# HybridRobotics/car-racing

Measured on AMD Instinct MI355X. Metric: NLP solves/sec (N=12, 6-state bicycle); p50 per-step solve latency, higher is better.
Workload: dtype f64

## Files before the change

### car-racing_amd/csrc/crx_api.hip

```cpp
#include <hip/hip_runtime.h>
#include <math.h>
#include <stdarg.h>
#include <stdio.h>
#include <string.h>

#include <dlfcn.h>

#include <chrono>
#include <mutex>
#include <vector>

#if __has_include(<rccl/rccl.h>)
#include <rccl/rccl.h>
#else
extern "C" {
typedef struct ncclComm* ncclComm_t;
typedef struct { char internal[128]; } ncclUniqueId;
typedef enum { ncclSuccess = 0 } ncclResult_t;
typedef enum { ncclInt8 = 0, ncclUint8 = 1, ncclInt32 = 2, ncclUint32 = 3, ncclInt64 = 4, ncclUint64 = 5, ncclFloat16 = 6, ncclFloat32 = 7, ncclFloat64 = 8 } ncclDataType_t;
}
#endif

#include "crx_kparams.h"

// ... 35 lines not shown
    }
    void release() {
        if (p) (void)hipFree(p);
        p = nullptr;
        cap = 0;
    }
};
DevBuf g_in, g_out;

struct PinBuf {
    void* p = nullptr;
    size_t cap = 0;
    int ensure(size_t bytes) {
        if (bytes <= cap) return 0;
        if (p) (void)hipHostFree(p);
        p = nullptr;
        cap = 0;
        size_t want = bytes + bytes / 2 + 256;
        hipError_t e = hipHostMalloc(&p, want, hipHostMallocDefault);
        if (e != hipSuccess) return fail(CRX_ERR_HIP, "hipHostMalloc(%zu): %s", want, hipGetErrorString(e));
        cap = want;
        return 0;
    }
    void release() {
        if (p) (void)hipHostFree(p);
        p = nullptr;
        cap = 0;
    }
};
PinBuf g_hin, g_hout;
DevBuf g_trace;
int g_poison = 0;
int g_kkt_unscaled = 0;
int g_spec = 0;
int g_trace_rows = 0, g_trace_problem = 0;

int ensure_init() {
    if (g_init) return 0;
    return fail(CRX_ERR_NOT_INIT, "crx_init() has not been called (or failed)");
}

struct Stage {
    size_t oi = 0, oo = 0;
    struct Back { void* host; size_t off, bytes; };
    Back backs[16];
    int nb = 0;
    int reserve(size_t bytes_in, size_t bytes_out) {
        bytes_in += 20 * 256; bytes_out += 20 * 256;
        if (int rc = g_in.ensure(bytes_in)) return rc;
        if (int rc = g_hin.ensure(bytes_in)) return rc;
        if (int rc = g_out.ensure(bytes_out)) return rc;
        return g_hout.ensure(bytes_out);
    }
    template <typename T>
    T* in(const T* src, size_t n) {
        oi = (oi + 255) & ~size_t(255);
        T* dev = (T*)((char*)g_in.p + oi);
        if (n) {
            if (src) memcpy((char*)g_hin.p + oi, src, n * sizeof(T)); else memset((char*)g_hin.p + oi, 0, n * sizeof(T));
        }
        oi += n * sizeof(T);
        return dev;
    }
    template <typename T>
    T* out(T* host, size_t n) {
        oo = (oo + 255) & ~size_t(255);
// ... 81 lines not shown
    memcpy(kp.wq, d->Q, sizeof(kp.wq)); kp.wr[0] = d->R[0]; kp.wr[1] = d->R[1];
    kp.w_dey = 0.0; kp.w_prog = 0.0; kp.w_slack = d->w_slack;
    kp.delta_max = d->delta_max; kp.a_max = d->a_max; kp.v_min = d->v_min; kp.v_max = d->v_max; kp.ey_max = d->ey_max;
    kp.alpha = d->alpha; kp.margin = d->margin; kp.l_sum = d->l_sum; kp.w_sum = d->w_sum;
    kp.dt_ref = 0.1; kp.fallback_gain = 1.1; kp.opts = d->opts;
    kp.slack_start = d->opts.slack_start;
    double ws[6] = {0, 0, 0, 0, 1, 0}, we[6] = {0, 0, 0, 0, 0, 1}, as = 0.0, ae = 0.0;
    kp.reach_s[0] = 0.0; kp.reach_gain[0] = 0.0;
    for (int j = 1; j <= d->N; j++) {
        double s0 = 0.0, s1 = 0.0, e0 = 0.0, e1 = 0.0, wn[6] = {0, 0, 0, 0, 0, 0}, en[6] = {0, 0, 0, 0, 0, 0};
        for (int i = 0; i < 6; i++) {
            s0 += ws[i] * d->B[i * 2]; s1 += ws[i] * d->B[i * 2 + 1];
            e0 += we[i] * d->B[i * 2]; e1 += we[i] * d->B[i * 2 + 1];
        }
        as += fabs(s0) * d->delta_max + fabs(s1) * d->a_max;
        ae += fabs(e0) * d->delta_max + fabs(e1) * d->a_max;
        kp.reach_s[j] = as; kp.reach_gain[j] = ae;
        for (int a = 0; a < 6; a++)
            for (int i = 0; i < 6; i++) { wn[a] += ws[i] * d->A[i * 6 + a]; en[a] += we[i] * d->A[i * 6 + a]; }
        memcpy(ws, wn, sizeof(ws)); memcpy(we, en, sizeof(we));
    }
    return 0;
}

int launch_solve(const crx_kparams& kp, int tmpl, hipStream_t st) {
    crx_kparams kq = kp;
    if (g_trace_rows != 0) { kq.trace = (double*)g_trace.p; kq.trace_problem = g_trace_problem; kq.trace_rows = g_trace_rows; }
    kq.poison = g_poison;
    kq.kkt_unscaled = g_kkt_unscaled;
    size_t lds = crx_solve_lds_bytes(kp.N, tmpl);
    if (lds > 160 * 1024) return fail(CRX_ERR_ARG, "N=%d with %d obstacles needs %zu B of LDS (> 160 KiB)", kp.N, tmpl, lds);
    const bool spec = tmpl == 1 && kq.mode == 1 && kq.degree == 6 && (kq.N == 12 || kq.N == 10) && g_spec > 0;
    kq.spec_idle = g_spec == 2;
    hipError_t e = spec ? crx_launch_solve_spec(kq, st) : crx_launch_solve(kq, tmpl, st);
    if (e != hipSuccess) return fail(CRX_ERR_HIP, "solver launch: %s", hipGetErrorString(e));
    return 0;
}

}

extern "C" {

int crx_version(void) { return CRX_VERSION; }

const char* crx_last_error(void) { return g_err; }

int crx_device_count(void) {
    int n = 0;
    if (hipGetDeviceCount(&n) != hipSuccess) return 0;
    return n;
}

int crx_init(int device) {
    std::lock_guard<std::mutex> lk(g_mu);
    int n = 0;
    hipError_t e = hipGetDeviceCount(&n);
    if (e != hipSuccess || n <= 0)
        return fail(CRX_ERR_NO_DEVICE, "no HIP device visible (%s); libcrx has no CPU back-end",
                    e == hipSuccess ? "count = 0" : hipGetErrorString(e));
    if (device < 0 || device >= n) return fail(CRX_ERR_ARG, "device %d outside [0,%d)", device, n);
    HIP_TRY(hipSetDevice(device));
    if (g_init && g_device == device) return CRX_OK;
    if (g_init && g_device >= 0) {
        (void)hipSetDevice(g_device);
        if (g_stream) { (void)hipStreamDestroy(g_stream); g_stream = nullptr; }
        g_in.release(); g_out.release(); g_hin.release(); g_hout.release(); g_trace.release();
// ... 9 lines not shown
void crx_shutdown(void) {
    std::lock_guard<std::mutex> lk(g_mu);
    if (!g_init) return;
    (void)hipSetDevice(g_device);
    g_in.release(); g_out.release(); g_hin.release(); g_hout.release(); g_trace.release();
    g_trace_rows = 0;
    if (g_stream) (void)hipStreamDestroy(g_stream);
    g_stream = nullptr;
    g_init = false; g_device = -1;
}

int crx_trace_enable(int problem, int rows) {
    if (int rc = ensure_init()) return rc;
    g_trace_rows = 0;
    const bool sub = rows < 0;
    if (rows < 0) rows = -rows;
    if (rows == 0) return CRX_OK;
    if (int rc = g_trace.ensure((size_t)rows * 16 * sizeof(double))) return rc;
    HIP_TRY(hipMemset(g_trace.p, 0, (size_t)rows * 16 * sizeof(double)));
    g_trace_rows = sub ? -rows : rows; g_trace_problem = problem;
    return CRX_OK;
}
int crx_trace_read(double* host, int rows) {
    { int cap = g_trace_rows < 0 ? -g_trace_rows : g_trace_rows; if (rows > cap) rows = cap; }
    HIP_TRY(hipDeviceSynchronize());
    HIP_TRY(hipMemcpy(host, g_trace.p, (size_t)rows * 16 * sizeof(double), hipMemcpyDeviceToHost));
    return CRX_OK;
}

void crx_debug_poison_lds(int enable) { g_poison = enable != 0; }

void crx_debug_speculation(int mode) { g_spec = mode < 0 ? 0 : (mode > 2 ? 1 : mode); }

void crx_debug_kkt_unscaled(int mode) { g_kkt_unscaled = (mode >= 0 && mode <= 4) ? mode : 0; }

int crx_debug_wave_reduce(const double* in, double* out) {
    if (int rc = ensure_init()) return rc;
    if (!in || !out) return fail(CRX_ERR_ARG, "NULL array argument");
    std::lock_guard<std::mutex> lk(g_mu);
    HIP_TRY(hipSetDevice(g_device));
    Stage sg;
    if (int rc = sg.reserve(256 * 8, 208 * 8)) return rc;
    double* din = sg.in(in, 256);
    double* dout = sg.out(out, 208);
    if (int rc = sg.up(g_stream)) return rc;
    hipError_t e = crx_launch_debug_reduce(din, dout, g_stream);
    if (e != hipSuccess) return fail(CRX_ERR_HIP, "debug reduce launch: %s", hipGetErrorString(e));
    return sg.down(g_stream);
}

long crx_debug_lds_bytes(int kind, int N, int n) {
    return kind == 0 ? (long)crx_solve_lds_bytes(N, n) : (long)crx_lmpc_lds_bytes(N, n);
}

int crx_debug_resident_per_cu(int kind, int N, int n) {
    if (ensure_init() != CRX_OK) return -1;
    return kind == 0 ? crx_solve_resident_per_cu(N, n) : crx_lmpc_resident_per_cu(N, n);
}

struct CrxTimer { hipEvent_t e0, e1; bool armed; };

int crx_timer_create(void** timer) {
    if (int rc = ensure_init()) return rc;
    if (!timer) return fail(CRX_ERR_ARG, "timer is NULL");
    HIP_TRY(hipSetDevice(g_device));
    CrxTimer* t = new CrxTimer{nullptr, nullptr, false};
    if (hipEventCreate(&t->e0) != hipSuccess || hipEventCreate(&t->e1) != hipSuccess) {
        if (t->e0) (void)hipEventDestroy(t->e0);
        delete t;
        return fail(CRX_ERR_HIP, "hipEventCreate failed");
    }
    *timer = t;
    return CRX_OK;
}
int crx_timer_destroy(void* timer) {
    CrxTimer* t = (CrxTimer*)timer;
    if (!t) return CRX_OK;
    (void)hipEventDestroy(t->e0); (void)hipEventDestroy(t->e1);
    delete t;
    return CRX_OK;
}
int crx_timer_begin(void* timer, void* stream) {
    CrxTimer* t = (CrxTimer*)timer;
    if (!t) return fail(CRX_ERR_ARG, "timer is NULL");
    t->armed = false;
    HIP_TRY(hipEventRecord(t->e0, (hipStream_t)stream));
    return CRX_OK;
}
int crx_timer_end(void* timer, void* stream) {
    CrxTimer* t = (CrxTimer*)timer;
// ... 1135 lines not shown
```

### car-racing_amd/csrc/crx_kernels.hip

```cpp
#include <hip/hip_runtime.h>
#include <math.h>
#include <stdint.h>
#include <type_traits>

#include "crx_kparams.h"
#include "crx_wave.h"

#ifndef CRX_KKT_DIAG
#define CRX_KKT_DIAG 1
#endif
#ifndef CRX_TU_GENERAL
#define CRX_TU_GENERAL 0
#endif
#ifndef CRX_OPAQUE_LANE
#define CRX_OPAQUE_LANE 1
#endif
#ifndef CRX_OPAQUE_OUTER
#define CRX_OPAQUE_OUTER 0
#endif
#ifndef CRX_W2_FLOOR
#define CRX_W2_FLOOR 0
#endif
#ifndef CRX_STATIC_LDS
#define CRX_STATIC_LDS 1
// ... 243 lines not shown
#define CLK() clock64()
#else
#define CLK() 0LL
#endif

template <int NOBS, int NMAX>
__device__ __forceinline__ void cbf_dist(const double* sm, const Ctx& c, int k, int o, double al, double& dsc,
                                         double& dec, double& dsn, double& den) {
    using L = Lay<NOBS, NMAX>;
    const int N1 = c.N + 1;
    const double sc = LD(L::Z + k * L::NZ + 4) + al * LD(L::dZ + k * L::NZ + 4);
    const double ec = LD(L::Z + k * L::NZ + 5) + al * LD(L::dZ + k * L::NZ + 5);
    const double sn = LD(L::Z + (k + 1) * L::NZ + 4) + al * LD(L::dZ + (k + 1) * L::NZ + 4);
    const double en = LD(L::Z + (k + 1) * L::NZ + 5) + al * LD(L::dZ + (k + 1) * L::NZ + 5);
    const double rLs = LD(L::cst + 16 + o), rWs = LD(L::cst + 16 + L::NO + o);
    dsc = (sc - LD(L::obs_s + o * N1 + k) - LD(L::cst + 8 + o)) * rLs;
    dec = (ec - LD(L::obs_e + o * N1 + k)) * rWs;
    dsn = (sn - LD(L::obs_s + o * N1 + k + 1)) * rLs;
    den = (en - LD(L::obs_e + o * N1 + k + 1)) * rWs;
}

template <int NOBS, int NMAX>
__device__ __forceinline__ double cbf_value(const double* sm, const Ctx& c, int k, int o, double al) {
    using L = Lay<NOBS, NMAX>;
    double dsc, dec, dsn, den;
    cbf_dist<NOBS, NMAX>(sm, c, k, o, al, dsc, dec, dsn, den);
    const int q = c.degree;
    const double gc = ipow_d(dsc, q) + ipow_d(dec, q), gn = ipow_d(dsn, q) + ipow_d(den, q);
    const double sk = LD(L::Z + k * L::NZ + 6 + o) + al * LD(L::dZ + k * L::NZ + 6 + o);
    const double sk1 = LD(L::Z + k * L::NZ + L::NX + 2 + o) + al * LD(L::dZ + k * L::NZ + L::NX + 2 + o);
    return gn - sk1 - c.om * (gc - sk) - c.alpha * c.cm;
}

template <int NOBS, int NMAX>
__device__ __forceinline__ double cost_value(const double* sm, const Ctx& c, double al) {
    using L = Lay<NOBS, NMAX>;
    const int N = c.N;
    double acc = 0.0;
    for (int e = c.lane; e < (N + 1) * 6; e += WAVE) {
        const int k = e / 6, i = e - k * 6;
        const double v = LD(L::Z + k * L::NZ + i) + al * LD(L::dZ + k * L::NZ + i);
        const double d = v - LD(L::xr + e);
        acc += LD(L::cst + i) * d * d;
        if (k == N && i == 4) acc += c.lin_sN * v;
    }
    for (int e = c.lane; e < N * 2; e += WAVE) {
        const int k = e >> 1, i = e & 1;
        const double v = LD(L::Z + k * L::NZ + L::NX + i) + al * LD(L::dZ + k * L::NZ + L::NX + i);
        acc += LD(L::cst + 6 + i) * v * v;
    }
    for (int k = c.lane; k < N; k += WAVE) {
        const double wck = LD(L::wc + k);
        const double e1 = LD(L::Z + (k + 1) * L::NZ + 5) + al * LD(L::dZ + (k + 1) * L::NZ + 5);
        const double e0 = LD(L::Z + k * L::NZ + 5) + al * LD(L::dZ + k * L::NZ + 5);
        acc += wck * (e1 - e0) * (e1 - e0);
    }
    if (NOBS) {
        for (int e = c.lane; e < (N + 1) * NOBS; e += WAVE) {
            const int k = e / L::NO, o = e - k * L::NO;
            if (o < c.nobs) acc += c.wsig * (LD(L::Z + k * L::NZ + 6 + o) + al * LD(L::dZ + k * L::NZ + 6 + o));
        }
    }
    return wave_sum(acc) + c.cconst;
}

template <int NOBS, int NMAX>
// ... 983 lines not shown
    SYNC();
    const double s0 = bs[0];
    for (int e = lane; e < (N + 1) * 6; e += WAVE) {
        const int j = e / 6, i = e - j * 6;
        const double st = s0 + kp.fallback_gain * j * kp.dt_ref * vx0;
        double v = 0.0;
        if (i == 0) v = kp.fallback_gain * vx0;
        else if (i == 4) v = st;
        else if (i == 5) v = interp_lin(bs, be, N + 1, fmin(fmax(st, bs[0]), bs[N]));
        Xb[e] = v;
    }
    for (int e = lane; e < N * 2; e += WAVE) Ub[e] = 0.0;
    if (lane == 0) kp.cost[b] = INFINITY;
}

#ifndef CRX_PLANNER_WAVES
#define CRX_PLANNER_WAVES 3
#endif
#ifndef CRX_OBS1_WAVES
#define CRX_OBS1_WAVES 2
#endif
#ifndef CRX_KERNEL_EXTRA_ATTR
#define CRX_KERNEL_EXTRA_ATTR
#endif
#ifndef CRX_GEN_WAVES
#define CRX_GEN_WAVES 0
#endif
template <int NOBS, int NMAX> struct MinWaves {
    static constexpr int v = CRX_GEN_WAVES ? CRX_GEN_WAVES : (((NOBS == 1 || (CRX_W2_FLOOR && NOBS == 2)) && NMAX == 12) ? CRX_OBS1_WAVES : ((NOBS == 0 && NMAX == 12) ? CRX_PLANNER_WAVES : 1));
};

template <int NFIX> struct SweepUnroll { static constexpr int v = NFIX == 0 ? 1 : (CRX_SWEEP_UNROLL ? NFIX : 2); };
template <int NOBS, int NFIX> struct RicUnroll { static constexpr int v = NFIX == 0 ? 1 : (CRX_RIC_UNROLL == 0 ? NFIX : CRX_RIC_UNROLL); };
template <int NOBS, int NMAX, int DEG = 0, int NFIX = 0, int SPEC = 0, int QPM = 0>
__global__ void __launch_bounds__(WAVE * (1 + SPEC)) __attribute__((amdgpu_waves_per_eu(MinWaves<NOBS, NMAX>::v))) CRX_KERNEL_EXTRA_ATTR
crx_solve_kernel(const crx_kparams kp) {
    static_assert(NFIX <= NMAX, "fixed horizon inside the layout");
    using L = Lay<NOBS, NMAX>;
    static_assert(!SPEC || (NOBS > 0 && !L::SLIM && CRX_STATIC_LDS), "the speculating wave exists for the obstacle instantiations of the full, static layout");
    constexpr int NX = L::NX, NZ = L::NZ, NR = L::NR;
#if CRX_STATIC_LDS
    __shared__ __attribute__((aligned(16))) double sm[((SPEC ? L::BYTES_SPEC : L::BYTES) + 7) / 8];
#else
    extern __shared__ __attribute__((aligned(16))) double sm[];
#endif
    int* si = (int*)(sm + L::END_D);
    const int lane = SPEC ? (int)(threadIdx.x & (WAVE - 1)) : (int)threadIdx.x, N = NFIX ? NFIX : kp.N;
    if ((int)blockIdx.x >= kp.batch) return;
    const int b = kp.order ? min(max(kp.order[blockIdx.x], 0), kp.batch - 1) : (int)blockIdx.x;
    if (kp.active && kp.active[kp.active_div > 1 ? b / kp.active_div : b] == 0) {
        if (lane == 0) { kp.status[b] = CRX_SKIPPED; kp.iters[b] = 0; }
        return;
    }
    if (NOBS == 0 && kp.mode == 0 && kp.reach_screen) {
        bool out = false;
        for (int j = lane; j < N; j += WAVE) {
            double fr = 0.0;
#pragma unroll
            for (int i = 0; i < 6; i++) fr += kp.reach_row[j][i] * kp.x0[(size_t)b * 6 + i];
            const double g = kp.reach_gain[j];
            out = out || kp.ey_lb[(size_t)b * N + j] > fr + g + 1e-6 || kp.ey_ub[b] < fr - g - 1e-6;
        }
        if (__ballot(out) != 0ull) {
            planner_fallback<L>(sm, kp, b, lane, N);
            if (lane == 0) { kp.status[b] = CRX_INFEASIBLE; kp.kkt[b] = INFINITY; kp.iters[b] = 0; }
            return;
        }
    }
    if constexpr (SPEC) {
        if (threadIdx.x >= WAVE) {
            Ctx c1 = {};
            c1.N = N; c1.lane = lane;
// ... 553 lines not shown
                    for (int e = lane; e < N * L::NU; e += WAVE) LD(L::kf + e) = LD(L::kf2 + e);
                    if (lane < NZ) LD(L::dZ + lane) = LD(L::dZ2 + lane);
                    SYNC();
                    ok = true; used_convex = ncz;
                    break;
                }
                sdw = ntries == 0 ? (dw_last == 0.0 ? 1e-4 : fmax(1e-20, dw_last / 3.0)) : ndw * (dw_last == 0.0 ? 100.0 : 8.0);
                cz = ncz; avail = 0; tries = ntries + 1;
                dw = sdw;
                if (sdw > 1e40) break;
            }
        } else
        for (int tries = 0, convex = (NOBS > 0 && crash && !used_convex) ? 0 : 1;; ) {
            ok = riccati_backward<NOBS, NMAX, RicUnroll<NOBS, NFIX>::v>(sm, si, c, dw, tsub);
            if (ok) break;
            if (NOBS && !convex) {
                used_convex = 1;
                convex = 1;
                for (int k = lane; k < N; k += WAVE) { LD(L::kS + 2 * k) = 0.0; LD(L::kE + 2 * k) = 0.0; }
                SYNC();
                continue;
            }
            dw = tries == 0 ? (dw_last == 0.0 ? 1e-4 : fmax(1e-20, dw_last / 3.0)) : dw * (dw_last == 0.0 ? 100.0 : 8.0);
            tries++;
            if (dw > 1e40) break;
        }
        if (!ok) break;
        if (dw != 0.0) dw_last = dw;
        cvx_run = used_convex ? cvx_run + 1 : 0;
        long long tc5 = CLK();
        riccati_forward<NOBS, NMAX, SweepUnroll<NFIX>::v>(sm, c);
        long long tc6 = CLK();
        double rp_max = 0.0, rd_max = 0.0, theta = 0.0, Dphi = 0.0;
        auto row_step = [&](int j, bool cnt, bool store, double sc, double jd) {
            const bool on = sc != 0.0;
            const double t = LD(L::rt + j), nu = LD(L::rnu + j), rti = LD(L::rtt + j), rcj = LD(L::rc + j);
            double rwj, rsj;
            row_sig_w<L>(sm, j, on, mu, t, nu, rti, rcj, rsj, rwj);
            ROW_LOADS_DONE();
            const double rp = rcj - t;
            const double dt = sel(on, jd + rp, 0.0);
            const double dnu = sel(on, -rwj + rsj * (rp - dt), 0.0);
            LD(SINK(store, L::rdt + j)) = dt;
            const double dtr = dt * rti;
            rp_max = fmax(rp_max, sel(cnt, -dtr, 0.0));
            rd_max = fmax(rd_max, sel(cnt && on, -dnu * frcp(nu), 0.0));
            theta += sel(cnt && on, fabs(rp), 0.0);
            Dphi -= sel(cnt && on, mu * dtr, 0.0);
        };
        ROWS(j, jv, lane, m) {
            const bool simple = !ROW_IS_CBF(j, N);
            const int pk = RIVT(si, j);
            const double sc = row_scale<L>(sm, si, j, N), jd = RIV_SGN(pk) * LD(L::dZ + RIV_IDX(pk));
            row_step(j, jv && simple, simple, sc, jd);
        }
        if (NOBS) {
            CBF_ROWS(j, k, ob, ev, lane, N) {
                const double* J = sm + L::Jc + (k * L::NO + ob) * NZ;
                double jc = 0.0;
#pragma unroll
                for (int a = 0; a < NZ; a++) jc += J[a] * LD(L::dZ + k * NZ + a);
                row_step(j, ev, true, cbf_scale<L>(sm, k, ob), jc);
            }
        }
        wave_max2(rp_max, rd_max);
        const double a_p = (rp_max > tau) ? tau / rp_max : 1.0;
        const double a_d = (rd_max > tau) ? tau / rd_max : 1.0;
        double cost_qq;
        double cost_d = cost_dir<NOBS, NMAX>(sm, c, cost_qq);
        wave_sum4(theta, Dphi, cost_d, cost_qq);
        Dphi += cost_d;
        const double phi0 = f - mu * logsum_t;
        if (theta_min < 0.0) {
            theta_min = 1e-4 * fmax(1.0, theta);
            theta_max = 1e4 * fmax(1.0, theta);
        }
        long long tc7 = CLK();
        double al = a_p, fn = f, lt_acc = logsum_t;
        int acc = 0, ftype = 0;
        const bool sw_try = (theta <= theta_min) && (Dphi < 0.0);
        const double sw_gap = sw_try ? 2.3 * log2_fast(-Dphi) - 1.1 * log2_fast(theta) : 0.0;
        for (int ls = 0; ls < 40 && al >= 1e-10; ls++) {
            fn = f + al * (cost_d + al * cost_qq);
            double thn = 0.0;
            LogAcc lg;
            auto row_trial = [&](int j, bool cnt, bool store, double sc, double cn, double t, double dt) {
                double tn = t + al * dt;
                tn = sel(cn > tn, cn, tn);
                const bool off = sc == 0.0;
                tn = sel(off, 1.0, tn);
                cn = sel(off, 1.0, cn);
                LD(SINK(store, L::rtt + j)) = tn;
                lg.mul(sel(cnt, tn, 1.0));
                thn += sel(cnt, fabs(cn - tn), 0.0);
            };
            ROWS(j, jv, lane, m) {
                const bool simple = !ROW_IS_CBF(j, N);
                const double sc = row_scale<L>(sm, si, j, N), t = LD(L::rt + j), dt = LD(L::rdt + j), cj = LD(L::rc + j);
                ROW_LOADS_DONE();
                row_trial(j, jv && simple, simple, sc, cj + al * (dt - (cj - t)), t, dt);
            }
            if (NOBS) {
                CBF_ROWS(j, k, ob, ev, lane, N) {
                    const double sc = cbf_scale<L>(sm, k, ob), t = LD(L::rt + j), dt = LD(L::rdt + j);
                    row_trial(j, ev, true, sc, sc * cbf_value<NOBS, NMAX>(sm, c, k, ob, al), t, dt);
                }
            }
            lt_acc = lg.wave_total_with(thn);
            const double phin = fn - mu * lt_acc;
            int okf = (thn <= theta_max) && (phin == phin);
            {
                const bool iv = lane < nf;
                const int i = iv ? lane : 0;
                const double fth = LD(L::Fth + i), fph = LD(L::Fph + i);
                if (__any(iv && !(thn < fth || phin < fph))) okf = 0;
            }
            if (okf) {
                if (sw_try && log2_fast(al) + sw_gap > 0.0) {
                    if (phin <= phi0 + eta * al * Dphi + 10.0 * 2.2e-16 * fabs(phi0)) { acc = 1; ftype = 1; }
                } else if (thn <= (1.0 - 1e-5) * theta || phin <= phi0 - 1e-8 * theta) {
                    acc = 1;
                }
            }
            if (acc) break;
            al *= 0.5;
        }
        long long tc8 = CLK();
        tph[0] = tc1 - tc0; tph[1] = tc2 - tc1; tph[2] = tc3 - tc2; tph[3] = tc4 - tc3; tph[4] = tc5 - tc4;
        tph[5] = tc6 - tc5; tph[6] = tc7 - tc6; tph[7] = tc8 - tc7;
        if (kp.trace_rows < 0) { tph[0] = tsub[0]; tph[1] = tsub[1]; tph[2] = tsub[2]; tph[3] = tsub[3]; }
        if (kp.trace && b == kp.trace_problem && it < (kp.trace_rows < 0 ? -kp.trace_rows : kp.trace_rows) && lane == 0) {
            double* tr = kp.trace + (size_t)it * 16;
            for (int q = 0; q < 8; q++) tr[8 + q] = (double)(tph[q]);
            tr[0] = e_d; tr[1] = e_p; tr[2] = e_c; tr[3] = mu; tr[4] = al; tr[5] = a_d; tr[6] = dw; tr[7] = acc ? (ftype ? 2.0 : 1.0) : 0.0;
        }
        if (acc && !ftype && nf < MAXF) {
            if (lane == 0) { LD(L::Fth + nf) = (1.0 - 1e-5) * theta; LD(L::Fph + nf) = phi0 - 1e-8 * theta; }
            nf++;
        }
        if (!acc) { ls_failed = 1; break; }
        if (NOBS) {
            jam = (jam_on && al < JAM_ALPHA && e_p > o.tol) ? jam + 1 : 0;
            if (jam_on && n_restore == 0 && it >= STALL_ITERS && e_p > 1e-6) jam = JAM_COUNT;
            if (jam >= JAM_COUNT && n_restore < 2) { ls_failed = 2; break; }
        }
        SYNC();
        COORDS(e, ev, lane, N * NZ + NX) {
            const double zn = LD(L::Z + e) + al * LD(L::dZ + e);
            LD(SINK(ev, L::Z + e)) = zn;
        }
        SYNC();
        f = fn;
        logsum_t = lt_acc;
        double numax = 0.0, th = 0.0;
        nus = 0.0; cmax = 0.0; cmin = INFINITY;
        auto row_accept = [&](int j, bool own, double sc, double v) {
            const bool on = sc != 0.0, cnt = own && on;
            const double tn = LD(L::rtt + j), rcj = LD(L::rc + j), rtj = LD(L::rt + j);
            const double rdj = LD(L::rdt + j), rnj = LD(L::rnu + j);
            double rwj, rsj;
            row_sig_w<L>(sm, j, on, mu, rtj, rnj, L::SLIM ? frcp(rtj) : 0.0, rcj, rsj, rwj);
            ROW_LOADS_DONE();
            const double mut = mu * frcp(tn);
            const double rp = rcj - rtj;
            const double dnu = -rwj + rsj * (rp - rdj);
            double nn = rnj + a_d * dnu;
            nn = fmin(fmax(nn, mut * (1.0 / kappa_sigma)), kappa_sigma * mut);
            LD(SINK(cnt, L::rt + j)) = tn;
            LD(SINK(cnt, L::rnu + j)) = nn;
            numax = fmax(numax, sel(cnt, nn, 0.0));
            th = fmax(th, sel(cnt, fabs(v - tn), 0.0));
            nus += sel(cnt, nn, 0.0);
            cmax = fmax(cmax, sel(cnt, tn * nn, 0.0));
            cmin = fmin(cmin, sel(cnt, tn * nn, INFINITY));
            LD(SINK(own, L::rc + j)) = sel(on, v, 1.0);
        };
        ROWS(j, jv, lane, m) {
            const int pk = RIVT(si, j);
            const double sc = row_scale<L>(sm, si, j, N), v = RIV_SGN(pk) * (LD(L::Z + RIV_IDX(pk)) - row_bound<L>(sm, c, j));
            row_accept(j, jv && !ROW_IS_CBF(j, N), sc, v);
        }
        if (NOBS) {
            CBF_ROWS(j, k, ob, ev, lane, N) {
                const double sc = cbf_scale<L>(sm, k, ob);
                row_accept(j, ev, sc, sc * cbf_value<NOBS, NMAX>(sm, c, k, ob, 0.0));
            }
        }
        SYNC();
        {
            double ncmin = -cmin;
            wave_max4(numax, th, cmax, ncmin);
            cmin = -ncmin;
        }
        nus = wave_sum(nus);
        e_p = th;
        first_order<NOBS, NMAX>(sm, si, c);
        if (kp.trace && b == kp.trace_problem && it < (kp.trace_rows < 0 ? -kp.trace_rows : kp.trace_rows) && lane == 0 && kp.trace_rows > 0)
            kp.trace[(size_t)it * 16 + 8] = (double)(tph[0] + (CLK() - tc8));
        if (numax > 1e12 && th > 1e-6) { status = CRX_STALLED; it++; break; }
        if (NOBS == 0 && th > 1e-6) {
            if (box_certificate<NOBS, NMAX>(sm, si, c, kp.delta_max, kp.a_max) < -1e-8 * numax) { status = 2; it++; break; }
        }
    }
    if (!ls_failed) break;
    int full = 0;
    if (NOBS && crash_path && n_restore == 0 && !crash && crash_cand >= 0) {
        crash_write<NOBS, NMAX, false>(sm, c, kp, crash_cand);
        crash = 1; full = 1;
    }
    if (NOBS && o.restore_iters >= 0 && n_restore < 2 && (__builtin_amdgcn_readfirstlane((int)restore_slacks<NOBS, NMAX>(sm, c, o.slack_push)) | full)) {
        eval_rows<NOBS, NMAX>(sm, si, c);
        SYNC();
        for (int j = lane; j < m; j += WAVE) {
            const bool cbf = ROW_IS_CBF(j, N);
            const int r = j < N * NR ? j % NR : 8;
            const bool sig = NOBS && (j >= N * NR || (r >= 8 && r < 8 + NOBS));
            if (row_scale<L>(sm, si, j, N) != 0.0) {
                const double t = fmax(fabs(LD(L::rc + j)), o.slack_push);
// ... 76 lines not shown
    int best = 0;
    for (int r = 0; r < R; r++) {
        double cst = INFINITY;
        if (r <= nv) {
            const double* Xr = sp.X + (((size_t)s * R + r) * (N + 1)) * 6;
            double hits = 0.0;
            for (int e = lane; e < 2 * (N + 1); e += WAVE) {
                const int side = e / (N + 1), j = e - side * (N + 1);
                const int v = side == 0 ? r - 1 : r;
                if (v < 0 || v >= nv) continue;
                double os = sp.obs_s[((size_t)s * V + v) * (N + 1) + j];
                os = wrap_above(os, sp.lap_length);
                const double ds = Xr[6 * j + 4] - os;
                const double de = Xr[6 * j + 5] - sp.obs_ey[((size_t)s * V + v) * (N + 1) + j];
                if (!(ds * ds + de * de - r2 >= 0.0)) hits += 1.0;
            }
            hits = wave_sum(hits);
            cst = -sp.w_prog * (Xr[6 * N + 4] - Xr[4]) + sp.w_coll * hits;
            if (sp.old_flag[s] >= 0 && sp.old_flag[s] != r) cst += sp.w_switch;
            if (cst < best_c) { best_c = cst; best = r; }
        }
        if (lane == 0) sp.sel_cost[(size_t)s * R + r] = cst;
    }
    if (lane == 0) sp.flag[s] = best;
    const double* Xb = sp.X + (((size_t)s * R + best) * (N + 1)) * 6;
    for (int e = lane; e < (N + 1) * 6; e += WAVE) sp.best_X[(size_t)s * (N + 1) * 6 + e] = Xb[e];
}

#endif

#ifdef CRX_PROBE_ONE
template __global__ void crx_solve_kernel<CRX_PROBE_ONE>(const crx_kparams);
#else
template <int NOBS, int NMAX, int DEG = 0, int NFIX = 0, int SPEC = 0, int QPM = 0>
static hipError_t launch_t(const crx_kparams& kp, hipStream_t st) {
    if constexpr (NOBS == 0 && QPM == 0) {
        if (kp.opts.qp_method != 0) return launch_t<NOBS, NMAX, DEG, NFIX, SPEC, 1>(kp, st);
    }
#if CRX_STATIC_LDS
    hipLaunchKernelGGL((crx_solve_kernel<NOBS, NMAX, DEG, NFIX, SPEC, QPM>), dim3(kp.batch), dim3(WAVE * (1 + SPEC)), 0, st, kp);
#else
    static_assert(SPEC == 0, "the two-wave instantiations are static-LDS kernels");
    const size_t bytes = Lay<NOBS, NMAX>::BYTES;
    static int attr_set_on = -1;
    int dev = -1;
    if (hipGetDevice(&dev) != hipSuccess) return hipErrorInvalidDevice;
    if (attr_set_on != dev) {
        hipError_t e = hipFuncSetAttribute((const void*)crx_solve_kernel<NOBS, NMAX, DEG, NFIX, 0, QPM>, hipFuncAttributeMaxDynamicSharedMemorySize, (int)bytes);
        if (e != hipSuccess) return e;
        attr_set_on = dev;
    }
    hipLaunchKernelGGL((crx_solve_kernel<NOBS, NMAX, DEG, NFIX, 0, QPM>), dim3(kp.batch), dim3(WAVE), bytes, st, kp);
#endif
    return hipGetLastError();
}
#ifdef CRX_TU_SPEC
hipError_t crx_launch_solve_spec(const crx_kparams& kp, hipStream_t st) {
    if (kp.batch == 0) return hipSuccess;
    if (kp.degree != 6) return hipErrorInvalidValue;
    if (kp.N == 12) return launch_t<1, 12, 6, 12, 1>(kp, st);
    if (kp.N == 10) return launch_t<1, 12, 6, 10, 1>(kp, st);
    return hipErrorInvalidValue;
}
#else
hipError_t crx_launch_solve_general(const crx_kparams& kp, int nobs_template, hipStream_t st);
int crx_solve_resident_per_cu_general(int N, int nobs_template);
#if !CRX_TU_GENERAL
#ifndef CRX_NFIX_LIST
#define CRX_NFIX_LIST 10, 12, 20
#endif
template <int NOBS, int NF> struct NfixLayout { static constexpr int v = NF <= 12 ? 12 : ((NOBS == 3 && NF <= 20) ? 20 : CRX_MAX_N); };
template <int NOBS, int DEG, int... NFS>
static bool launch_fixed(const crx_kparams& kp, hipStream_t st, hipError_t& e) {
    bool hit = false;
    (void)((kp.N == NFS ? (e = launch_t<NOBS, NfixLayout<NOBS, NFS>::v, DEG, NFS>(kp, st), hit = true) : false) || ...);
    return hit;
}
template <int NOBS>
static hipError_t launch_n(const crx_kparams& kp, hipStream_t st) {
    hipError_t e = hipSuccess;
    (void)e;
#if CRX_NFIX
    if constexpr (NOBS > 0 && CRX_DEG6) {
        if (kp.degree == 6 && launch_fixed<NOBS, 6, CRX_NFIX_LIST>(kp, st, e)) return e;
    } else {
        if (launch_fixed<NOBS, 0, CRX_NFIX_LIST>(kp, st, e)) return e;
    }
#endif
    return crx_launch_solve_general(kp, NOBS, st);
// ... 87 lines not shown
        case 1: return occ_g<1>(N);
        case 2: return occ_g<2>(N);
        case 3: return occ_g<3>(N);
        default: return N <= 12 ? occ_t<6, 12, 0>() : occ_t<6, CRX_MAX_N, 0>();
    }
}
#else
template <int NOBS, int... NFS>
static bool occ_fixed(int N, int& n) {
    bool hit = false;
    (void)((N == NFS ? (n = occ_t<NOBS, NfixLayout<NOBS, NFS>::v, NFS>(), hit = true) : false) || ...);
    return hit;
}
template <int NOBS>
static int occ_n(int N) {
#if CRX_NFIX
    int n = 0;
    if (occ_fixed<NOBS, CRX_NFIX_LIST>(N, n)) return n;
#endif
    return crx_solve_resident_per_cu_general(N, NOBS);
}
#endif
#if CRX_TU_GENERAL
#elif defined(CRX_TU_OBSTACLES)
int crx_solve_resident_per_cu_obs(int N, int nobs_template) {
    switch (nobs_template) {
        case 1: return occ_n<1>(N);
        case 2: return occ_n<2>(N);
        case 3: return occ_n<3>(N);
        default: return crx_solve_resident_per_cu_general(N, nobs_template);
    }
}
#else
int crx_solve_resident_per_cu(int N, int nobs_template) {
    return nobs_template == 0 ? occ_n<0>(N) : crx_solve_resident_per_cu_obs(N, nobs_template);
}

hipError_t crx_launch_select(const crx_select_kparams& sp, hipStream_t st) {
    if (sp.n_scen == 0) return hipSuccess;
    hipLaunchKernelGGL(crx_select_kernel, dim3(sp.n_scen), dim3(WAVE), 0, st, sp);
    return hipGetLastError();
}

__global__ void __launch_bounds__(WAVE) crx_debug_reduce_kernel(const double* in, double* out) {
    const int lane = threadIdx.x;
    double a = in[lane], b = in[64 + lane], c = in[128 + lane], d = in[192 + lane];
    double s0 = a, s1 = b, s2 = c, s3 = d;
    wave_sum4(s0, s1, s2, s3);
    double m0 = a, m1 = b, m2 = c, m3 = d;
    wave_max4(m0, m1, m2, m3);
    double p0 = a, p1 = b;
    wave_sum2(p0, p1);
    double q0 = c, q1 = d;
    wave_max2(q0, q1);
    int ex;
    const double r0 = wave_sum(a), r1 = wave_max(b), r2 = wave_min(c), r3 = wave_prod(frexp(fabs(d) + 1.0, &ex));
    if (lane == 0) {
        out[0] = s0; out[1] = s1; out[2] = s2; out[3] = s3; out[4] = m0; out[5] = m1; out[6] = m2; out[7] = m3;
        out[8] = p0; out[9] = p1; out[10] = q0; out[11] = q1; out[12] = r0; out[13] = r1; out[14] = r2; out[15] = r3;
    }
    double m[7];
#pragma unroll
    for (int i = 0; i < 7; i++) m[i] = (double)(i + 1) * b + d;
    out[16 + lane] = row_dot<7, 0>(a, m, c);
    double masked = __longlong_as_double(0x7ff8000000000000LL), chained = masked;
    if (lane < 10) {
        masked = row_dot<7, 3>(a, m, c);
// ... 15 lines not shown
```

### car-racing_amd/csrc/crx_kparams.h

```cpp
#ifndef CRX_KPARAMS_H
#define CRX_KPARAMS_H
#include <stdint.h>

#include "../../include/crx.h"

struct crx_kparams {
    int N, batch, mode , per_stage_target, n_obs_max, degree;
    double A[36], B[12];
    double wq[6], wr[2];
    double w_dey, w_prog, w_slack;
    double delta_max, a_max, v_min, v_max, ey_max;
    double alpha, margin, l_sum, w_sum;
    double dt_ref, fallback_gain;
    crx_ipm_opts opts;
    const double *x0, *bez_s, *bez_ey, *ey_lb, *ey_ub;
    const double *xt, *obs_s, *obs_ey, *lap_off;
    const int32_t* n_obs;
    const double* obs_dims;
    double *X, *U, *sigma, *cost, *kkt;
    int32_t *status, *iters;
    double* trace;
    int trace_problem, trace_rows;
    int poison;
    int kkt_unscaled;
    int spec_idle;
    const int32_t* active;
    int active_div;
    const int32_t* order;
    int reach_screen;
    double reach_gain[CRX_MAX_N + 1];
    double reach_row[CRX_MAX_N][6];
    int slack_start;
    double reach_s[CRX_MAX_N + 1];
};

struct crx_lmpc_kparams {
    int N, batch, n_ss_max;
    double Q[6], R[2], dR[2], x_track[6];
    double v_max, ey_max, delta_max, a_max, w_x0;
    crx_ipm_opts opts;
    const double *x0, *u_old, *A, *B, *C, *ss, *qfun;
    const int32_t* n_ss;
    double *X, *U, *lambda, *cost, *kkt;
    int32_t *status, *iters;
    double* trace;
    int trace_problem, trace_rows;
    int poison;
    const int32_t* active;
    const int32_t* order;
    int reach_screen;
};

struct crx_select_kparams {
    int N, V, n_scen;
    double veh_length, veh_width, lap_length, w_prog, w_coll, w_switch;
    const int32_t* n_veh;
    const double *X, *obs_s, *obs_ey;
    const int32_t* old_flag;
// ... 38 lines not shown
struct crx_trackprep_kparams {
    int N, V, batch;
    double lap_length, safety_time, dt_ref;
    const double *x, *obs_s_in, *obs_ey_in, *traj;
    const int32_t* n_veh;
    double *xt, *obs_s, *obs_ey, *lap_off;
    int32_t* n_obs;
};

struct crx_scene_kparams {
    crx_scene_desc d;
    int n_scen;
    const double *ego_xcurv, *veh_xcurv, *pred_s, *pred_ey;
    const int32_t* n_all;
    int32_t *n_veh, *overflow, *order;
    double *veh_info, *max_dv, *obs_s, *obs_ey;
};

struct crx_lmpcprep_kparams {
    crx_lmpcprep_desc d;
    int batch, from_plan;
    const double *ss_xcurv, *u_ss, *qfun;
    const int32_t *time_ss, *iter;
    const double *x, *lin_points, *lin_input, *track;
    double *A, *B, *C, *ss_sel, *q_sel;
    int32_t* status;
    const int32_t* active;
};

#ifdef __HIPCC__
#include <hip/hip_runtime.h>
hipError_t crx_launch_solve(const crx_kparams& kp, int nobs_template, hipStream_t st);
hipError_t crx_launch_solve_spec(const crx_kparams& kp, hipStream_t st);
hipError_t crx_launch_select(const crx_select_kparams& sp, hipStream_t st);
hipError_t crx_launch_debug_reduce(const double* in, double* out, hipStream_t st);
hipError_t crx_launch_lmpc_addtraj(const crx_lmpcprep_desc& d, int batch, const int32_t* crossed, double* log_x, const double* log_u,
                                   int32_t* n_log, double* ss_xcurv, double* u_ss, double* qfun, int32_t* time_ss, int32_t* iter,
                                   int32_t* step, const double* x, int32_t* status, hipStream_t st);
size_t crx_solve_lds_bytes(int N, int nobs_template);
int crx_solve_resident_per_cu(int N, int nobs_template);
hipError_t crx_launch_path(const crx_path_kparams& pp, hipStream_t st);
hipError_t crx_launch_cbfprep(const crx_cbfprep_kparams& cp, hipStream_t st);

struct crx_order_kparams {
    int batch, mode;
    const int32_t *iters, *active;
    int32_t* order;
    int V, stride, degree, per_stage_target;
    double margin, l_sum, w_sum, ds_per_vx;
    const double *x0, *xt, *obs_s, *obs_ey, *lap_off, *obs_dims;
    const int32_t* n_obs;
};
hipError_t crx_launch_order(const crx_order_kparams& op, hipStream_t st);

struct crx_game_kparams {
    int N, Np, batch, n_cars, n_points;
    double lap_length, t, dt;
    const double *car_s0, *car_v, *car_ey;
    double *veh_xcurv, *pred_s, *pred_ey;
    const int32_t *n_veh, *overflow;
    int32_t *m_overtake, *m_lmpc, *overflow_seen;
    const int32_t* overtake;
    const double *U_track, *X_lmpc, *U_lmpc;
    const int32_t* flag;
    double *u, *u_old, *u_prev, *lin_points, *lin_input;
    int32_t *step_no, *addpoint_step, *old_flag;
    const double* xcurv;
    const int32_t* laps;
    int32_t *laps_prev, *n_log, *crossed;
    double *log_x, *log_u;
};
hipError_t crx_launch_game(int which, const crx_game_kparams& gp, hipStream_t st);
hipError_t crx_launch_plant(const crx_plant_kparams& pk, hipStream_t st);
// ... 26 lines not shown
```

Measured before the change: 582,400.

## Add lone-wave solver variant that keeps row state in registers for small batches

```diff
diff --git a/car-racing_amd/csrc/crx_api.hip b/car-racing_amd/csrc/crx_api.hip
--- a/car-racing_amd/csrc/crx_api.hip
+++ b/car-racing_amd/csrc/crx_api.hip
@@ -91,6 +91,8 @@
 DevBuf g_trace;
 int g_poison = 0;
 int g_kkt_unscaled = 0;
+int g_lone = 0;
+int g_obs1_lone = 0;
 int g_spec = 0;
 int g_trace_rows = 0, g_trace_problem = 0;
 
@@ -238,6 +240,8 @@
     if (lds > 160 * 1024) return fail(CRX_ERR_ARG, "N=%d with %d obstacles needs %zu B of LDS (> 160 KiB)", kp.N, tmpl, lds);
     const bool spec = tmpl == 1 && kq.mode == 1 && kq.degree == 6 && (kq.N == 12 || kq.N == 10) && g_spec > 0;
     kq.spec_idle = g_spec == 2;
+    kq.lone_wave = g_lone;
+    if (tmpl == 1 && kq.N == 12 && kq.degree == 6 && !spec) g_obs1_lone = crx_solve_takes_lone(kq);
     hipError_t e = spec ? crx_launch_solve_spec(kq, st) : crx_launch_solve(kq, tmpl, st);
     if (e != hipSuccess) return fail(CRX_ERR_HIP, "solver launch: %s", hipGetErrorString(e));
     return 0;
@@ -313,6 +317,9 @@
 
 void crx_debug_speculation(int mode) { g_spec = mode < 0 ? 0 : (mode > 2 ? 1 : mode); }
 
+void crx_debug_lone_wave(int mode) { g_lone = (mode >= 0 && mode <= 2) ? mode : 0; }
+long crx_debug_lone_wave_launches() { return crx_solve_lone_launches(); }
+
 void crx_debug_kkt_unscaled(int mode) { g_kkt_unscaled = (mode >= 0 && mode <= 4) ? mode : 0; }
 
 int crx_debug_wave_reduce(const double* in, double* out) {
@@ -336,7 +343,13 @@
 
 int crx_debug_resident_per_cu(int kind, int N, int n) {
     if (ensure_init() != CRX_OK) return -1;
-    return kind == 0 ? crx_solve_resident_per_cu(N, n) : crx_lmpc_resident_per_cu(N, n);
+    return kind == 0 ? crx_solve_resident_per_cu(N, n, n == 1 && N == 12 && g_obs1_lone) : crx_lmpc_resident_per_cu(N, n);
+}
+int crx_debug_resident_per_cu_batch(int kind, int N, int n, int batch) {
+    if (ensure_init() != CRX_OK) return -1;
+    crx_kparams kq{};
+    kq.batch = batch; kq.lone_wave = g_lone;
+    return kind == 0 ? crx_solve_resident_per_cu(N, n, n == 1 && N == 12 && crx_solve_takes_lone(kq)) : crx_lmpc_resident_per_cu(N, n);
 }
 
 struct CrxTimer { hipEvent_t e0, e1; bool armed; };
diff --git a/car-racing_amd/csrc/crx_kernels.hip b/car-racing_amd/csrc/crx_kernels.hip
--- a/car-racing_amd/csrc/crx_kernels.hip
+++ b/car-racing_amd/csrc/crx_kernels.hip
@@ -299,6 +299,42 @@
     return gn - sk1 - c.om * (gc - sk) - c.alpha * c.cm;
 }
 
+struct RowReg {
+    double t, nu, rti, c, sig, w, sc, dt;
+    double tn;
+};
+struct CbfReg {
+    double zs, dzs, ze, dze, zs1, dzs1, ze1, dze1;
+    double os, oe, os1, oe1, lap, rLs, rWs;
+    double sg, dsg, sg1, dsg1;
+};
+template <int NOBS, int NMAX>
+__device__ __forceinline__ void cbf_load(const double* sm, const Ctx& c, int k, int o, CbfReg& r) {
+    using L = Lay<NOBS, NMAX>;
+    const int N1 = c.N + 1;
+    r.zs = LD(L::Z + k * L::NZ + 4); r.dzs = LD(L::dZ + k * L::NZ + 4);
+    r.ze = LD(L::Z + k * L::NZ + 5); r.dze = LD(L::dZ + k * L::NZ + 5);
+    r.zs1 = LD(L::Z + (k + 1) * L::NZ + 4); r.dzs1 = LD(L::dZ + (k + 1) * L::NZ + 4);
+    r.ze1 = LD(L::Z + (k + 1) * L::NZ + 5); r.dze1 = LD(L::dZ + (k + 1) * L::NZ + 5);
+    r.rLs = LD(L::cst + 16 + o); r.rWs = LD(L::cst + 16 + L::NO + o);
+    r.os = LD(L::obs_s + o * N1 + k); r.lap = LD(L::cst + 8 + o); r.oe = LD(L::obs_e + o * N1 + k);
+    r.os1 = LD(L::obs_s + o * N1 + k + 1); r.oe1 = LD(L::obs_e + o * N1 + k + 1);
+    r.sg = LD(L::Z + k * L::NZ + 6 + o); r.dsg = LD(L::dZ + k * L::NZ + 6 + o);
+    r.sg1 = LD(L::Z + k * L::NZ + L::NX + 2 + o); r.dsg1 = LD(L::dZ + k * L::NZ + L::NX + 2 + o);
+}
+__device__ __forceinline__ double cbf_eval(const Ctx& c, const CbfReg& r, double al) {
+    const double sc = fma(al, r.dzs, r.zs), ec = fma(al, r.dze, r.ze);
+    const double sn = fma(al, r.dzs1, r.zs1), en = fma(al, r.dze1, r.ze1);
+    const double dsc = (sc - r.os - r.lap) * r.rLs;
+    const double dec = (ec - r.oe) * r.rWs;
+    const double dsn = (sn - r.os1) * r.rLs;
+    const double den = (en - r.oe1) * r.rWs;
+    const int q = c.degree;
+    const double gc = ipow_d(dsc, q) + ipow_d(dec, q), gn = ipow_d(dsn, q) + ipow_d(den, q);
+    const double sk = fma(al, r.dsg, r.sg), sk1 = fma(al, r.dsg1, r.sg1);
+    return gn - sk1 - c.om * (gc - sk) - c.alpha * c.cm;
+}
+
 template <int NOBS, int NMAX>
 __device__ __forceinline__ double cost_value(const double* sm, const Ctx& c, double al) {
     using L = Lay<NOBS, NMAX>;
@@ -1348,12 +1384,14 @@
 
 template <int NFIX> struct SweepUnroll { static constexpr int v = NFIX == 0 ? 1 : (CRX_SWEEP_UNROLL ? NFIX : 2); };
 template <int NOBS, int NFIX> struct RicUnroll { static constexpr int v = NFIX == 0 ? 1 : (CRX_RIC_UNROLL == 0 ? NFIX : CRX_RIC_UNROLL); };
-template <int NOBS, int NMAX, int DEG = 0, int NFIX = 0, int SPEC = 0, int QPM = 0>
-__global__ void __launch_bounds__(WAVE * (1 + SPEC)) __attribute__((amdgpu_waves_per_eu(MinWaves<NOBS, NMAX>::v))) CRX_KERNEL_EXTRA_ATTR
+template <int NOBS, int NMAX, int DEG = 0, int NFIX = 0, int SPEC = 0, int QPM = 0, int LONE = 0>
+__global__ void __launch_bounds__(WAVE * (1 + SPEC)) __attribute__((amdgpu_waves_per_eu(LONE ? 1 : MinWaves<NOBS, NMAX>::v))) CRX_KERNEL_EXTRA_ATTR
 crx_solve_kernel(const crx_kparams kp) {
     static_assert(NFIX <= NMAX, "fixed horizon inside the layout");
     using L = Lay<NOBS, NMAX>;
     static_assert(!SPEC || (NOBS > 0 && !L::SLIM && CRX_STATIC_LDS), "the speculating wave exists for the obstacle instantiations of the full, static layout");
+    static_assert(!LONE || (NOBS > 0 && NOBS * NMAX <= WAVE && !SPEC && !L::SLIM), "the lone-wave form: obstacle instantiations of the full layout, one CBF pass");
+    constexpr bool LW = LONE != 0;
     constexpr int NX = L::NX, NZ = L::NZ, NR = L::NR;
 #if CRX_STATIC_LDS
     __shared__ __attribute__((aligned(16))) double sm[((SPEC ? L::BYTES_SPEC : L::BYTES) + 7) / 8];
@@ -1973,7 +2011,9 @@
         riccati_forward<NOBS, NMAX, SweepUnroll<NFIX>::v>(sm, c);
         long long tc6 = CLK();
         double rp_max = 0.0, rd_max = 0.0, theta = 0.0, Dphi = 0.0;
-        auto row_step = [&](int j, bool cnt, bool store, double sc, double jd) {
+        RowReg rr[(L::MR + WAVE - 1) / WAVE], rcb;
+        CbfReg cb;
+        auto row_step = [&](int j, bool cnt, bool store, double sc, double jd, RowReg& R) {
             const bool on = sc != 0.0;
             const double t = LD(L::rt + j), nu = LD(L::rnu + j), rti = LD(L::rtt + j), rcj = LD(L::rc + j);
             double rwj, rsj;
@@ -1981,6 +2021,7 @@
             ROW_LOADS_DONE();
             const double rp = rcj - t;
             const double dt = sel(on, jd + rp, 0.0);
+            if constexpr (LW) { R.t = t; R.nu = nu; R.rti = rti; R.c = rcj; R.sig = rsj; R.w = rwj; R.sc = sc; R.dt = dt; }
             const double dnu = sel(on, -rwj + rsj * (rp - dt), 0.0);
             LD(SINK(store, L::rdt + j)) = dt;
             const double dtr = dt * rti;
@@ -1993,7 +2034,7 @@
             const bool simple = !ROW_IS_CBF(j, N);
             const int pk = RIVT(si, j);
             const double sc = row_scale<L>(sm, si, j, N), jd = RIV_SGN(pk) * LD(L::dZ + RIV_IDX(pk));
-            row_step(j, jv && simple, simple, sc, jd);
+            row_step(j, jv && simple, simple, sc, jd, rr[q_]);
         }
         if (NOBS) {
             CBF_ROWS(j, k, ob, ev, lane, N) {
@@ -2001,7 +2042,8 @@
                 double jc = 0.0;
 #pragma unroll
                 for (int a = 0; a < NZ; a++) jc += J[a] * LD(L::dZ + k * NZ + a);
-                row_step(j, ev, true, cbf_scale<L>(sm, k, ob), jc);
+                row_step(j, ev, true, cbf_scale<L>(sm, k, ob), jc, rcb);
+                if constexpr (LW) cbf_load<NOBS, NMAX>(sm, c, k, ob, cb);
             }
         }
         wave_max2(rp_max, rd_max);
@@ -2025,26 +2067,36 @@
             fn = f + al * (cost_d + al * cost_qq);
             double thn = 0.0;
             LogAcc lg;
-            auto row_trial = [&](int j, bool cnt, bool store, double sc, double cn, double t, double dt) {
+            auto row_trial = [&](int j, bool cnt, bool store, double sc, double cn, double t, double dt, RowReg& R) {
                 double tn = t + al * dt;
                 tn = sel(cn > tn, cn, tn);
                 const bool off = sc == 0.0;
                 tn = sel(off, 1.0, tn);
                 cn = sel(off, 1.0, cn);
-                LD(SINK(store, L::rtt + j)) = tn;
+                if constexpr (LW) R.tn = tn;
+                else LD(SINK(store, L::rtt + j)) = tn;
                 lg.mul(sel(cnt, tn, 1.0));
                 thn += sel(cnt, fabs(cn - tn), 0.0);
             };
             ROWS(j, jv, lane, m) {
                 const bool simple = !ROW_IS_CBF(j, N);
-                const double sc = row_scale<L>(sm, si, j, N), t = LD(L::rt + j), dt = LD(L::rdt + j), cj = LD(L::rc + j);
-                ROW_LOADS_DONE();
-                row_trial(j, jv && simple, simple, sc, cj + al * (dt - (cj - t)), t, dt);
+                if constexpr (LW) {
+                    const RowReg& R = rr[q_];
+                    row_trial(j, jv && simple, simple, R.sc, R.c + al * (R.dt - (R.c - R.t)), R.t, R.dt, rr[q_]);
+                } else {
+                    const double sc = row_scale<L>(sm, si, j, N), t = LD(L::rt + j), dt = LD(L::rdt + j), cj = LD(L::rc + j);
+                    ROW_LOADS_DONE();
+                    row_trial(j, jv && simple, simple, sc, cj + al * (dt - (cj - t)), t, dt, rr[q_]);
+                }
             }
             if (NOBS) {
                 CBF_ROWS(j, k, ob, ev, lane, N) {
-                    const double sc = cbf_scale<L>(sm, k, ob), t = LD(L::rt + j), dt = LD(L::rdt + j);
-                    row_trial(j, ev, true, sc, sc * cbf_value<NOBS, NMAX>(sm, c, k, ob, al), t, dt);
+                    if constexpr (LW) {
+                        row_trial(j, ev, true, rcb.sc, rcb.sc * cbf_eval(c, cb, al), rcb.t, rcb.dt, rcb);
+                    } else {
+                        const double sc = cbf_scale<L>(sm, k, ob), t = LD(L::rt + j), dt = LD(L::rdt + j);
+                        row_trial(j, ev, true, sc, sc * cbf_value<NOBS, NMAX>(sm, c, k, ob, al), t, dt, rcb);
+                    }
                 }
             }
             lt_acc = lg.wave_total_with(thn);
@@ -2095,12 +2147,16 @@
         logsum_t = lt_acc;
         double numax = 0.0, th = 0.0;
         nus = 0.0; cmax = 0.0; cmin = INFINITY;
-        auto row_accept = [&](int j, bool own, double sc, double v) {
+        auto row_accept = [&](int j, bool own, double sc, double v, const RowReg& R) {
             const bool on = sc != 0.0, cnt = own && on;
-            const double tn = LD(L::rtt + j), rcj = LD(L::rc + j), rtj = LD(L::rt + j);
-            const double rdj = LD(L::rdt + j), rnj = LD(L::rnu + j);
-            double rwj, rsj;
-            row_sig_w<L>(sm, j, on, mu, rtj, rnj, L::SLIM ? frcp(rtj) : 0.0, rcj, rsj, rwj);
+            double tn, rcj, rtj, rdj, rnj, rwj, rsj;
+            if constexpr (LW) {
+                tn = R.tn; rcj = R.c; rtj = R.t; rdj = R.dt; rnj = R.nu; rsj = R.sig; rwj = R.w;
+            } else {
+                tn = LD(L::rtt + j); rcj = LD(L::rc + j); rtj = LD(L::rt + j);
+                rdj = LD(L::rdt + j); rnj = LD(L::rnu + j);
+                row_sig_w<L>(sm, j, on, mu, rtj, rnj, L::SLIM ? frcp(rtj) : 0.0, rcj, rsj, rwj);
+            }
             ROW_LOADS_DONE();
             const double mut = mu * frcp(tn);
             const double rp = rcj - rtj;
@@ -2118,13 +2174,16 @@
         };
         ROWS(j, jv, lane, m) {
             const int pk = RIVT(si, j);
-            const double sc = row_scale<L>(sm, si, j, N), v = RIV_SGN(pk) * (LD(L::Z + RIV_IDX(pk)) - row_bound<L>(sm, c, j));
-            row_accept(j, jv && !ROW_IS_CBF(j, N), sc, v);
+            const double sc = LW ? rr[q_].sc : row_scale<L>(sm, si, j, N), v = RIV_SGN(pk) * (LD(L::Z + RIV_IDX(pk)) - row_bound<L>(sm, c, j));
+            row_accept(j, jv && !ROW_IS_CBF(j, N), sc, v, rr[q_]);
         }
         if (NOBS) {
             CBF_ROWS(j, k, ob, ev, lane, N) {
-                const double sc = cbf_scale<L>(sm, k, ob);
-                row_accept(j, ev, sc, sc * cbf_value<NOBS, NMAX>(sm, c, k, ob, 0.0));
+                if constexpr (LW) row_accept(j, ev, rcb.sc, rcb.sc * cbf_value<NOBS, NMAX>(sm, c, k, ob, 0.0), rcb);
+                else {
+                    const double sc = cbf_scale<L>(sm, k, ob);
+                    row_accept(j, ev, sc, sc * cbf_value<NOBS, NMAX>(sm, c, k, ob, 0.0), rcb);
+                }
             }
         }
         SYNC();
@@ -2267,13 +2326,23 @@
 #ifdef CRX_PROBE_ONE
 template __global__ void crx_solve_kernel<CRX_PROBE_ONE>(const crx_kparams);
 #else
+template <int NOBS, int NMAX, int DEG, int NFIX> constexpr bool HAS_LONE = NOBS == 1 && NMAX == 12 && DEG == 6 && NFIX == 12 && CRX_STATIC_LDS;
 template <int NOBS, int NMAX, int DEG = 0, int NFIX = 0, int SPEC = 0, int QPM = 0>
 static hipError_t launch_t(const crx_kparams& kp, hipStream_t st) {
     if constexpr (NOBS == 0 && QPM == 0) {
         if (kp.opts.qp_method != 0) return launch_t<NOBS, NMAX, DEG, NFIX, SPEC, 1>(kp, st);
     }
+#ifndef CRX_TU_LONE
+    if constexpr (HAS_LONE<NOBS, NMAX, DEG, NFIX> && SPEC == 0) {
+        if (crx_solve_takes_lone(kp)) return crx_launch_solve_lone(kp, st);
+    }
+#endif
 #if CRX_STATIC_LDS
+#ifdef CRX_TU_LONE
+    hipLaunchKernelGGL((crx_solve_kernel<NOBS, NMAX, DEG, NFIX, SPEC, QPM, 1>), dim3(kp.batch), dim3(WAVE), 0, st, kp);
+#else
     hipLaunchKernelGGL((crx_solve_kernel<NOBS, NMAX, DEG, NFIX, SPEC, QPM>), dim3(kp.batch), dim3(WAVE * (1 + SPEC)), 0, st, kp);
+#endif
 #else
     static_assert(SPEC == 0, "the two-wave instantiations are static-LDS kernels");
     const size_t bytes = Lay<NOBS, NMAX>::BYTES;
@@ -2289,7 +2358,37 @@
 #endif
     return hipGetLastError();
 }
-#ifdef CRX_TU_SPEC
+#ifdef CRX_TU_LONE
+static long g_lone_launches = 0;
+hipError_t crx_launch_solve_lone(const crx_kparams& kp, hipStream_t st) {
+    if (kp.batch == 0) return hipSuccess;
+    if (kp.degree != 6 || kp.N != 12) return hipErrorInvalidValue;
+    g_lone_launches++;
+    return launch_t<1, 12, 6, 12>(kp, st);
+}
+long crx_solve_lone_launches() { return g_lone_launches; }
+bool crx_solve_takes_lone(const crx_kparams& kp) {
+    return kp.lone_wave == 1 || (kp.lone_wave == 0 && kp.batch <= crx_solve_lone_slots());
+}
+int crx_solve_lone_slots() {
+    static int slots[64] = {0};
+    int dev = -1;
+    if (hipGetDevice(&dev) != hipSuccess || dev < 0) return 0;
+    if (dev >= 64) dev = 63;
+    if (slots[dev] == 0) {
+        int cus = 0;
+        if (hipDeviceGetAttribute(&cus, hipDeviceAttributeMultiprocessorCount, dev) != hipSuccess || cus <= 0) return 0;
+        slots[dev] = 4 * cus;
+    }
+    return slots[dev];
+}
+int crx_solve_resident_per_cu_lone(int N) {
+    int n = 0;
+    if (N != 12) return -1;
+    if (hipOccupancyMaxActiveBlocksPerMultiprocessor(&n, crx_solve_kernel<1, 12, 6, 12, 0, 0, 1>, WAVE, 0) != hipSuccess) return -1;
+    return n;
+}
+#elif defined(CRX_TU_SPEC)
 hipError_t crx_launch_solve_spec(const crx_kparams& kp, hipStream_t st) {
     if (kp.batch == 0) return hipSuccess;
     if (kp.degree != 6) return hipErrorInvalidValue;
@@ -2443,7 +2542,8 @@
     }
 }
 #else
-int crx_solve_resident_per_cu(int N, int nobs_template) {
+int crx_solve_resident_per_cu(int N, int nobs_template, bool lone) {
+    if (lone && nobs_template == 1 && N == 12 && CRX_DEG6 && CRX_NFIX) return crx_solve_resident_per_cu_lone(N);
     return nobs_template == 0 ? occ_n<0>(N) : crx_solve_resident_per_cu_obs(N, nobs_template);
 }
 
diff --git a/car-racing_amd/csrc/crx_kernels_lone.hip b/car-racing_amd/csrc/crx_kernels_lone.hip
--- /dev/null
+++ b/car-racing_amd/csrc/crx_kernels_lone.hip
@@ -0,0 +1,3 @@
+#define CRX_TU_OBSTACLES 1
+#define CRX_TU_LONE 1
+#include "crx_kernels.hip"
diff --git a/car-racing_amd/csrc/crx_kparams.h b/car-racing_amd/csrc/crx_kparams.h
--- a/car-racing_amd/csrc/crx_kparams.h
+++ b/car-racing_amd/csrc/crx_kparams.h
@@ -24,6 +24,7 @@
     int poison;
     int kkt_unscaled;
     int spec_idle;
+    int lone_wave;
     const int32_t* active;
     int active_div;
     const int32_t* order;
@@ -128,13 +129,18 @@
 #include <hip/hip_runtime.h>
 hipError_t crx_launch_solve(const crx_kparams& kp, int nobs_template, hipStream_t st);
 hipError_t crx_launch_solve_spec(const crx_kparams& kp, hipStream_t st);
+hipError_t crx_launch_solve_lone(const crx_kparams& kp, hipStream_t st);
+int crx_solve_lone_slots();
+int crx_solve_resident_per_cu_lone(int N);
+long crx_solve_lone_launches();
 hipError_t crx_launch_select(const crx_select_kparams& sp, hipStream_t st);
 hipError_t crx_launch_debug_reduce(const double* in, double* out, hipStream_t st);
 hipError_t crx_launch_lmpc_addtraj(const crx_lmpcprep_desc& d, int batch, const int32_t* crossed, double* log_x, const double* log_u,
                                    int32_t* n_log, double* ss_xcurv, double* u_ss, double* qfun, int32_t* time_ss, int32_t* iter,
                                    int32_t* step, const double* x, int32_t* status, hipStream_t st);
 size_t crx_solve_lds_bytes(int N, int nobs_template);
-int crx_solve_resident_per_cu(int N, int nobs_template);
+int crx_solve_resident_per_cu(int N, int nobs_template, bool lone = false);
+bool crx_solve_takes_lone(const crx_kparams& kp);
 hipError_t crx_launch_path(const crx_path_kparams& pp, hipStream_t st);
 hipError_t crx_launch_cbfprep(const crx_cbfprep_kparams& cp, hipStream_t st);
 
```

New measurement: 596,600 (median of 6 runs). 2.4% higher.
